# h-walk/PySlice

Hardware: AMD Instinct MI355X
Metric: slice-steps/sec (probes x frames x slices / s), potential + slice loop + exit FFT (higher is better)
Workload: dtype complex64 (f32); 1 GPU; 64-probe STEM grid, 1024x1024 grid, 200 slices, 54 MD frames per GPU (BASELINE configs[2] per-frame work), 106583 atoms, 30 mrad, 100 keV; grid=1024, slices=200, probes=64, parallelism=frames x1, world_size_checked=1, frame_slots=59, frame_batch=4

## Files before the change

pyslice_amd/csrc/mslice.hip:

```cpp
#include <hip/hip_runtime.h>

#include <algorithm>
#include <cmath>
#include <cstdarg>
#include <cstdio>
#include <cstdlib>
#include <cstring>
#include <string>
#include <vector>

#include "../../include/mslice.h"
#include "fft_generic.h"
#include "fft_pow2.h"
#include "rowtm_pass.h"
#include "potential.h"
#include "thermal.h"
#include "reduce.h"
#include "stream.h"
#include "tacaw_time.h"
#include "tacaw_launch.h"
#include "tacaw_welch.h"
#include "layer_tap.h"
#include "detect.h"
#include "spectrum_detect.h"
// ... 1196 lines not shown
    }
    switch (o.base) {
    case AX_TWO: {
        std::vector<float2> t(o.R * o.R);
        for (int m = 0; m < o.R * o.R; ++m) {
            const double a = -2.0 * M_PI * (double)m / (double)n;
            t[m] = make_float2((float)cos(a), (float)sin(a));
        }
        if ((rc = make_tw4(h, o.tw, o.R)) || (rc = upload(h, o.tw2, t)) || (rc = o.ptab.alloc(h, (size_t)n))) return rc;
        break;
    }
    case AX_WAVE2K:
        if ((rc = make_wave2k_tables(h, o.tw, o.tw2))) return rc;
        break;
    case AX_CONV:
    case AX_CONV2K:
        if ((rc = make_cz_tables(h, o.cz, n)) || (rc = o.qf.alloc(h, conv_filter_entries(o)))) return rc;
        break;
    case AX_CONV4K: {
        std::vector<float2> wq(2048);
        for (int i = 0; i < 2048; ++i) {
            const double a = -2.0 * M_PI * (double)i / 4096.0;
            wq[i] = make_float2((float)cos(a), (float)sin(a));
        }
        if ((rc = make_wave2k_tables(h, o.tw, o.tw2)) || (rc = upload(h, o.bw, wq)) || (rc = o.qf.alloc(h, conv_filter_entries(o)))) return rc;
        break;
    }
    default:
        break;
    }
    auto conv = [](const msl_handle::OpDir& d) { return d.base == AX_CONV || d.base == AX_CONV2K; };
    if (!conv(o) && conv(other) && n >= 33 && n <= 1024) return make_cz_tables(h, o.cz, n);
    return MSL_OK;
}

PotIfft plan_pot_ifft(const msl_handle* h) {
    if (!h->onepass || h->V) return PI_LINES;
    if (h->opx.base == AX_WAVE2K && h->opy.base == AX_WAVE2K && h->transT) return PI_WAVE2K;
    if (h->transT && h->opx.cz.R && h->opy.cz.R) return PI_CHIRPZ;
    if (h->opx.base == AX_TWO && h->opy.base == AX_TWO) return PI_TWO;
    return PI_LINES;
}

bool pot_half_rows(const msl_handle* h) { return h->pot_ifft != PI_LINES || (h->Rx && h->Ry); }

struct PotGroup {
    int z2s[104], species[104], nsp;
    int64_t n; int32_t ax1, ax2, axs;
    int keys_per_frame;
    int cx, cy; float vscale;
    bool half_rows, sf_stream;
    int g, slot, n_slices, nkeys;
    long long rows, rows_pad;
    float2* TR; float2* TRT;
};

int map_species(msl_handle* h, const int32_t* Z, int64_t n, PotGroup& m) {
    for (int i = 0; i < 104; ++i) m.z2s[i] = -1;
    for (int64_t a = 0; a < n; ++a) {
        if (Z[a] < 1 || Z[a] > 103) return fail(h, MSL_ERR_INVALID, "msl_build_potential: atomic number %d out of 1..103", Z[a]);
        m.z2s[Z[a]] = 0;
    }
    m.nsp = 0;
    for (int z = 1; z <= 103; ++z) if (m.z2s[z] == 0) { m.z2s[z] = m.nsp; m.species[m.nsp++] = z; }
    return MSL_OK;
}

int stage_atoms(msl_handle* h, const PotGroup& p, const double* pos, const int32_t* Z, bool send_maps) {
    msl_handle::HostStage& st = h->stage[h->stage_pos++ & 1];
    if (!st.ev) HIPCHK(h, hipEventCreateWithFlags(&st.ev, hipEventDisableTiming));
    if (st.used) HIPCHK(h, hipEventSynchronize(st.ev));
    const size_t z_bytes = (size_t)p.n * sizeof(int), pos_bytes = (size_t)p.rows * 3 * sizeof(double);
    const size_t off_sp = sizeof p.z2s, off_Z = (off_sp + sizeof p.species + 7) & ~(size_t)7;
    const size_t off_pos = (off_Z + z_bytes + 7) & ~(size_t)7, need = off_pos + pos_bytes;
    if (need > st.bytes) {
        if (st.buf) (void)hipHostFree(st.buf);
        st.buf = nullptr; st.bytes = 0;
        const size_t cap = need + need / 4;
        if (hipHostMalloc((void**)&st.buf, cap, hipHostMallocDefault) != hipSuccess)
            return fail(h, MSL_ERR_NOMEM, "hipHostMalloc(%zu bytes) failed", cap);
        st.bytes = cap;
    }
    memcpy(st.buf + off_pos, pos, pos_bytes);
    if (send_maps) {
        memcpy(st.buf, p.z2s, sizeof p.z2s);
        memcpy(st.buf + off_sp, p.species, sizeof p.species);
        memcpy(st.buf + off_Z, Z, z_bytes);
        HIPCHK(h, hipMemcpyAsync(h->d_z2s, st.buf, sizeof p.z2s, hipMemcpyHostToDevice, h->stream));
        HIPCHK(h, hipMemcpyAsync(h->d_species, st.buf + off_sp, p.nsp * sizeof(int), hipMemcpyHostToDevice, h->stream));
        HIPCHK(h, hipMemcpyAsync(h->d_Z, st.buf + off_Z, z_bytes, hipMemcpyHostToDevice, h->stream));
    }
    HIPCHK(h, hipMemcpyAsync(h->d_pos, st.buf + off_pos, pos_bytes, hipMemcpyHostToDevice, h->stream));
    HIPCHK(h, hipEventRecord(st.ev, h->stream));
    st.used = true;
    return MSL_OK;
}

struct ThermalSource { uint64_t seed; uint64_t first_config; };

int stage_thermal(msl_handle* h, const PotGroup& p, uint64_t seed, uint64_t first_config, bool send_maps) {
    if (send_maps) {
        HIPCHK(h, hipMemcpyAsync(h->d_z2s, h->th_z2s, sizeof p.z2s, hipMemcpyDeviceToDevice, h->stream));
        HIPCHK(h, hipMemcpyAsync(h->d_species, h->th_species, p.nsp * sizeof(int), hipMemcpyDeviceToDevice, h->stream));
        HIPCHK(h, hipMemcpyAsync(h->d_Z, h->th_Z, (size_t)p.n * sizeof(int), hipMemcpyDeviceToDevice, h->stream));
    }
    hipLaunchKernelGGL(thermal_positions_kernel, dim3((unsigned)((p.rows + 255) / 256)), dim3(256), 0, h->stream, h->th_pos0, h->th_sigma,
                       (long long)p.n, p.g, (unsigned long long)seed, (unsigned long long)first_config, h->d_pos);
    HIPCHK(h, hipGetLastError());
    return MSL_OK;
}

int bin_atoms(msl_handle* h, const PotGroup& p) {
    const msl_config& c = h->cfg;
    const int nsp = p.nsp;
    HIPCHK(h, hipMemsetAsync(h->d_counts, 0, ((size_t)p.nkeys + 1) * sizeof(int), h->stream));
    const double lx = c.nx * c.dx, ly = c.ny * c.dy;
    if (nsp != h->ff_n || memcmp(p.species, h->ff_species, nsp * sizeof(int)) != 0) {
        long long tot = (long long)c.nx * c.ny * nsp;
        hipLaunchKernelGGL(formfactor_kernel, dim3((unsigned)((tot + 255) / 256)), dim3(256), 0, h->stream, h->d_ff, h->d_abcd,
                           h->d_species, nsp, c.nx, c.ny, 1.0 / lx, 1.0 / ly);
        memcpy(h->ff_species, p.species, nsp * sizeof(int));
        h->ff_n = nsp;
    }
    hipLaunchKernelGGL(atom_prep_kernel, dim3((unsigned)((p.rows + 255) / 256)), dim3(256), 0, h->stream, h->d_pos, h->d_Z,
                       (long long)p.n, p.g, h->d_z2s, h->d_lo, h->d_hi, c.nz, nsp, p.ax1, p.ax2, p.axs, 1.0 / lx, 1.0 / ly, h->d_key,
                       h->d_u1, h->d_u2, h->d_counts);
    hipLaunchKernelGGL(bin_scan_kernel, dim3(1), dim3(1024), 0, h->stream, h->d_counts, h->d_start, p.nkeys, p.sf_stream ? SF_ALIGN : 1);
    hipLaunchKernelGGL(bin_fill_kernel, dim3(p.nkeys), dim3(1024), 0, h->stream, h->d_key, (long long)p.n, p.keys_per_frame, h->d_start, h->d_order);
    HIPCHK(h, hipGetLastError());
    const int* n_sorted = h->d_start + p.nkeys;
    if (p.rows_pad > 0x7fffffffLL) return fail(h, MSL_ERR_INVALID, "msl_build_potentials: %lld padded table rows in one group exceed 2^31", p.rows_pad);
    const long long tx = p.rows_pad * p.cx, ty = p.rows_pad * p.cy;
    hipLaunchKernelGGL(phase_table_kernel, dim3((unsigned)((tx + 255) / 256)), dim3(256), 0, h->stream, h->d_ex, h->d_u1,
                       h->d_order, n_sorted, c.nx, p.cx, p.cx);
    hipLaunchKernelGGL(phase_table_kernel, dim3((unsigned)((ty + 255) / 256)), dim3(256), 0, h->stream, h->d_ey, h->d_u2,
                       h->d_order, n_sorted, c.ny, p.cy, p.cy);
    return MSL_OK;
}

int launch_structure_factor(msl_handle* h, const PotGroup& p) {
    const msl_config& c = h->cfg;
    const int cx = p.cx, cy = p.cy, nsp = p.nsp, n_slices = p.n_slices, full_rows = p.half_rows ? 0 : 1;
    const bool edge_x = (c.nx % 2 == 0) && (cx % 32 == 1) && cx > 1, edge_y = (c.ny % 2 == 0) && (cy % 32 == 1) && cy > 1;
    const int tiles_x = edge_x ? cx / 32 : (cx + 31) / 32, tiles_y = edge_y ? cy / 32 : (cy + 31) / 32;
    const int n_tiles = tiles_x * tiles_y, wg_per_slice = (n_tiles + 3) / 4;
    const long long n_wg = (long long)wg_per_slice * ((n_slices + 7) / 8 * 8);
    if (n_wg > 0x7fffffffLL) return fail(h, MSL_ERR_UNSUPPORTED, "structure factor: too many workgroups");
    if (p.sf_stream) {
        const int n_pers = std::max(8, h->n_cus / 8 * 8);
        auto stream = [&](auto kernel, size_t lds, int tiles) {
            hipLaunchKernelGGL(kernel, dim3((unsigned)n_pers), dim3(256), lds, h->stream, p.TR, h->d_ex, h->d_ey, h->d_ff, h->d_start, nsp,
                               c.nx, c.ny, tiles_y, tiles, (int)p.rows_pad, full_rows, cx, cy, n_slices);
        };
        if (dbg_env("MSL_SF_F32"))
            stream(structure_factor_stream_kernel, 0, n_tiles);
        else if ((n_tiles >= 512 || (tiles_x >= 2 && dbg_env("MSL_SF_TWO_TILES"))) && !dbg_env("MSL_SF_ONE_TILE"))
            stream(structure_factor_stream_bf16x2_kernel, 4 * 128 * 64 * sizeof(float), ((tiles_x + 1) / 2) * tiles_y);
        else
            stream(structure_factor_stream_bf16_kernel, 0, n_tiles);
    } else
        hipLaunchKernelGGL(structure_factor_quad_kernel, dim3((unsigned)n_wg), dim3(256), 0, h->stream, p.TR, h->d_ex, h->d_ey, h->d_ff,
                           h->d_start, nsp, c.nx, c.ny, tiles_y, n_tiles, (int)p.rows_pad, full_rows, cx, cy, n_slices, wg_per_slice);
    if (edge_x || edge_y) {
        const int bins = (edge_x ? cy : 0) + (edge_y ? (edge_x ? cx - 1 : cx) : 0);
        for (int s0 = 0; s0 < n_slices; s0 += 65535) {
            const int ns = std::min(65535, n_slices - s0);
            hipLaunchKernelGGL(structure_factor_edge_kernel, dim3((bins + 127) / 128, ns), dim3(128), 0, h->stream,
                               p.TR + (size_t)s0 * c.nx * c.ny, h->d_ex, h->d_ey, h->d_ff, h->d_start + (size_t)s0 * nsp, nsp, c.nx, c.ny,
                               edge_x ? 1 : 0, edge_y ? 1 : 0, full_rows, cx, cy);
        }
    }
    HIPCHK(h, hipGetLastError());
    return MSL_OK;
}

int launch_ifftTW(msl_handle* h, const msl_handle::OpDir& o, IfftTBJob j) {
    constexpr int N2 = 2048;
    const size_t lds = ((size_t)N2 + 64 + (size_t)8 * (N2 + 1)) * 8;
    const long long items = (long long)(j.n_lines / 8) * j.n_images;
    const int grid = (int)std::min<long long>(items, (long long)h->n_cus);
    j.tw = o.tw; j.tw2 = o.tw2;
    return launch_lds(h, ifftTW_kernel, dim3(grid), dim3(512), lds, K_OTHER, j);
}

int launch_ifftTB(msl_handle* h, const msl_handle::OpDir& o, IfftTBJob j) {
    const CzTables& t = o.cz;
    j.tw = t.tw; j.bf = t.bf; j.bw = t.bw;
    if (t.R == 64) {
        constexpr int M2 = 2048, NH2 = 1024, RS = (32 * W2K_PITCH) / 2 + 1;
        const size_t lds2 = ((size_t)M2 + 64 + NH2 + 2 + NH2 + (size_t)8 * RS) * 8;
        const long long items2 = (long long)((j.n_lines + 7) / 8) * j.n_images;
        const int grid2 = (int)std::min<long long>(items2, (long long)h->n_cus);
        j.tw2 = t.tw2;
        return launch_lds(h, ifftTB2_kernel, dim3(grid2), dim3(512), lds2, K_OTHER, j);
    }
    const int R = t.R, M = R * R, NH = M / 2, CS = R * (R + 1) + 2;
    const size_t lds = ((size_t)M + NH + 2 + NH + (size_t)16 * CS) * 8;
    const int per_cu = std::max(1, std::min(R == 16 ? 4 : 1, (int)((size_t)h->lds_limit / lds)));
    if (R == 32 && !j.potential && !dbg_env("MSL_NO_TWO_LINE_IFFT")) {
        constexpr int CSN = 514;
        const size_t lds2 = ((size_t)M + NH + 2 + NH + (size_t)32 * CSN) * 8;
        const long long items2 = (long long)((j.n_lines + 31) / 32) * j.n_images;
        const int grid2 = (int)std::min<long long>(items2, (long long)h->n_cus);
        return launch_lds(h, ifftTB_two_kernel, dim3(grid2), dim3(512), lds2, K_OTHER, j);
    }
    const bool pair = R == 32 && j.herm && j.potential && !dbg_env("MSL_NO_PAIRED_IFFT");
    const long long items = (long long)((j.n_lines + (pair ? 31 : 15)) / (pair ? 32 : 16)) * j.n_images;
    const dim3 grid((unsigned)std::min<long long>(items, (long long)h->n_cus * per_cu));
    if (pair) return launch_lds(h, ifftTB_kernel<32, true>, grid, dim3(512), lds, K_OTHER, j);
    if (R == 32) return launch_lds(h, ifftTB_kernel<32>, grid, dim3(512), lds, K_OTHER, j);
    return launch_lds(h, ifftTB_kernel<16>, grid, dim3(256), lds, K_OTHER, j);
}

int launch_ifftT2(msl_handle* h, const msl_handle::OpDir& o, IfftT2Job j) {
    constexpr int R = 16, N2 = R * R, N = 2 * N2;
    const size_t lds = ((size_t)2 * N2 + (size_t)16 * (N + 1)) * 8;
    const int per_cu = std::max(1, std::min(2, (int)((size_t)h->lds_limit / lds)));
    const bool pair = j.herm && j.potential && j.n_lines % 32 == 0 && !dbg_env("MSL_NO_PAIRED_IFFT");
    const long long items = (long long)(j.n_lines / (pair ? 32 : 16)) * j.n_images;
    const dim3 grid((unsigned)std::min<long long>(items, (long long)h->n_cus * per_cu));
    j.tw = o.tw; j.tw2 = o.tw2;
    if (pair) return launch_lds(h, ifftT2_kernel<16, true>, grid, dim3(256), lds, K_OTHER, j);
    return launch_lds(h, ifftT2_kernel<16>, grid, dim3(256), lds, K_OTHER, j);
}

template <typename Job>
int ifft_transposed(msl_handle* h, const PotGroup& p, int line_block, int (*launch)(msl_handle*, const msl_handle::OpDir&, Job)) {
    const msl_config& c = h->cfg;
    const long long npix = (long long)c.nx * c.ny;
    Job a{};
    a.in = p.TR; a.out_t = p.TRT; a.out_rows = nullptr;
    a.in_is = a.out_t_is = npix; a.in_pitch = c.ny; a.out_t_pitch = c.nx; a.n_images = p.n_slices;
    a.n_lines = (c.nx / 2 + 1 + line_block - 1) / line_block * line_block;
    a.potential = 0; a.rows_parity = -1; a.slice_mod = c.nz;
    Job b{};
    b.in = p.TRT; b.out_t = p.TR; b.out_rows = p.TRT;
    b.in_is = b.out_t_is = b.out_rows_is = npix; b.in_pitch = c.nx; b.out_t_pitch = c.ny; b.out_rows_pitch = c.nx;
    b.n_lines = c.ny; b.n_images = p.n_slices; b.potential = 1; b.herm = 1; b.slice_mod = c.nz;
    b.rows_parity = slice_is_transposed(h, 1) ? 1 : 0;
    b.scale = p.vscale; b.sigma_over_pi = (float)(c.sigma / M_PI);
    if constexpr (std::is_same<Job, IfftTBJob>::value) { a.n_line = c.ny; b.n_line = c.nx; }
    const int rc = launch(h, h->opy, a);
    return rc ? rc : launch(h, h->opx, b);
}

int ifft_inplace(msl_handle* h, const PotGroup& p) {
    const msl_config& c = h->cfg;
    int rc;
    if (h->Ry) {
        RowJob r = row_job(h, p.TR, p.n_slices, c.ny);
        r.do_ifft = 1;
        if (p.half_rows) { const int Gr = 256 / h->Ry; r.nx = (c.nx / 2 + 1 + Gr - 1) / Gr * Gr; }
        if ((rc = launch_row_fast(h, r, K_OTHER))) return rc;
    } else {
        LineArgs r = row_args(h, p.TR, p.TR, p.n_slices, c.ny);
        r.fft1 = -1;
        if ((rc = launch_lines(h, h->plan_y, r, K_OTHER))) return rc;
    }
    if (h->Rx) {
        ColJob k = col_job(h, p.TR, p.TR, p.n_slices, c.ny, c.ny);
        k.flags = COL_INV | COL_POTENTIAL; k.scale = p.vscale; k.sigma = (float)c.sigma; k.out_real = h->V; k.slice_mod = c.nz;
        if (h->onepass && !h->V) { k.flags |= COL_TPOT; k.tparity = h->scheme_b ? 0 : ((c.nz - 1) & 1); k.out_t = p.TRT; }
        if ((rc = p.half_rows ? launch_col_herm(h, k, K_OTHER) : launch_col_fast(h, k, K_OTHER))) return rc;
        return (h->onepass && h->V) ? transpose_odd_slices(h, p.slot) : MSL_OK;
    }
    LineArgs k = col_args(h, p.TR, p.TR, p.n_slices, c.ny, c.ny);
    k.fft1 = -1; k.scale = p.vscale;
    k.store_mode = STORE_POTENTIAL; k.out_real = h->V; k.sigma = (float)c.sigma;
    if ((rc = launch_lines(h, h->plan_x, k, K_OTHER))) return rc;
    for (int f = 0; f < p.g && rc == MSL_OK; ++f) rc = transpose_odd_slices(h, p.slot + f);
    return rc;
}

int potential_ifft(msl_handle* h, const PotGroup& p) {
    h->cur = nullptr;
    switch (h->pot_ifft) {
    case PI_WAVE2K: return ifft_transposed(h, p, 8, launch_ifftTW);
    case PI_CHIRPZ: return ifft_transposed(h, p, 1, launch_ifftTB);
    case PI_TWO:    return ifft_transposed(h, p, 16, launch_ifftT2);
    default:        return ifft_inplace(h, p);
    }
}

int build_potentials(msl_handle* h, const double* pos, const int32_t* Z, int64_t n, int count, int first_slot, int32_t ax1, int32_t ax2, int32_t axs,
                     const ThermalSource* th = nullptr) {
    const msl_config& c = h->cfg;
    const size_t npix = (size_t)c.nx * c.ny;
    PotGroup p{};
    int rc = MSL_OK;
    if (th) {
        memcpy(p.z2s, h->th_map_z2s, sizeof p.z2s);
        memcpy(p.species, h->th_map_species, sizeof p.species);
        p.nsp = h->th_nsp;
    } else {
        rc = map_species(h, Z, n, p);
    }
    if (rc) return rc;
    EventPair timer;
    if (c.launch_timing && (rc = timer.begin(h))) return rc;
    if (p.nsp > h->ff_species_cap) {
        if ((rc = h->d_ff.alloc(h, npix * p.nsp))) return rc;
        h->ff_species_cap = p.nsp;
        h->ff_n = 0;
    }
    p.n = n; p.ax1 = ax1; p.ax2 = ax2; p.axs = axs;
    p.cx = c.nx / 2 + 1; p.cy = c.ny / 2 + 1; p.keys_per_frame = c.nz * std::max(p.nsp, 1);
    p.half_rows = pot_half_rows(h);
    p.sf_stream = (double)n / std::max(1, p.keys_per_frame) >= 128.0 && !dbg_env("MSL_SF_TILED");
    p.vscale = (float)(1.0 / ((double)c.nx * c.ny) / (c.dx * c.dx * c.dy * c.dy));
// ... 1803 lines not shown
```

pyslice_amd/csrc/potential.h:

```cpp
#pragma once
#include <hip/hip_runtime.h>
#include <stdint.h>
#include "kernel_util.h"

namespace msl {

__device__ __forceinline__ int signed_freq(int m, int n) { return (m < (n + 1) / 2) ? m : m - n; }

__global__ void formfactor_kernel(float* __restrict__ ff, const double* __restrict__ abcd,
                                  const int* __restrict__ species, int n_species, int nx, int ny,
                                  double inv_lx, double inv_ly) {
    long long i = (long long)blockIdx.x * blockDim.x + threadIdx.x;
    long long npix = (long long)nx * ny;
    if (i >= npix * n_species) return;
    int sp = (int)(i / npix);
    long long p = i - (long long)sp * npix;
    int mx = (int)(p / ny), my = (int)(p - (long long)mx * ny);
    double kx = signed_freq(mx, nx) * inv_lx, ky = signed_freq(my, ny) * inv_ly;
    double q2 = kx * kx + ky * ky;
    const double* t = abcd + (size_t)(species[sp] - 1) * 12;
    double s1 = 0.0, s2 = 0.0;
#pragma unroll
    for (int j = 0; j < 3; ++j) {
        s1 += t[j * 4 + 0] / (q2 + t[j * 4 + 1]);
// ... 349 lines not shown
                x[u] = make_float2(a.x, a.y); y[u] = make_float2(b.x, b.y);
            }
        };
        auto mma = [&](f32x16& acc, const sf_u32x4& a, const sf_u32x4& b) { asm volatile("v_mfma_f32_32x32x16_bf16 %0, %1, %2, %0" : "+a"(acc) : "v"(a), "v"(b)); };
        auto mma6 = [&](f32x16& acc, const sf_u32x4 (&p)[3], const sf_u32x4 (&q)[3]) {
            mma(acc, p[0], q[0]); mma(acc, p[0], q[1]); mma(acc, p[1], q[0]);
            mma(acc, p[0], q[2]); mma(acc, p[2], q[0]); mma(acc, p[1], q[1]);
        };
        auto conv = [&](sf_u32x4 (&o)[3], const float2 (&v)[8], bool imag) {
#pragma unroll
            for (int u = 0; u < 4; ++u) {
                unsigned p0, p1, p2;
                sf_split3(imag ? v[2 * u].y : v[2 * u].x, imag ? v[2 * u + 1].y : v[2 * u + 1].x, p0, p1, p2);
                o[0][u] = p0; o[1][u] = p1; o[2][u] = p2;
            }
        };
        sf_u32x4 cx[3], sx[3], cy[3], sy[3];
        auto trip = [&](int h, float2 (&x)[8], float2 (&y)[8], const float2 (&xn)[8], const float2 (&yn)[8]) {
            if (S0 + 16 * h == seg1) flush();
            mma6(A, cx, cy); conv(sy, y, true); conv(sx, x, true); __builtin_amdgcn_sched_barrier(0);
            load16(h + 2, x, y); __builtin_amdgcn_sched_barrier(0);
            mma6(C, cx, sy); conv(cx, xn, false); __builtin_amdgcn_sched_barrier(0);
            mma6(D, sx, cy); conv(cy, yn, false); __builtin_amdgcn_sched_barrier(0);
            mma6(B, sx, sy); __builtin_amdgcn_sched_barrier(0);
        };
        float2 x0[8], y0[8], x1[8], y1[8];
        if (H > 0) { load16(0, x0, y0); load16(1, x1, y1); conv(cx, x0, false); conv(cy, y0, false); }
        for (int h = 0; h < H; h += 2) {
            trip(h, x0, y0, x1, y1);
            if (h + 1 < H) trip(h + 1, x1, y1, x0, y0);
        }
        if (H > 0) flush();
        float2* out = recip + (size_t)s * nx * ny;
        const int my = ky0 + i;
        if (my > hy) continue;
#pragma unroll
        for (int r = 0; r < 16; ++r) {
            const int mx = kx0 + (r & 3) + 8 * (r >> 2) + 4 * kk;
            if (mx > hx) continue;
            store_quad_bin(out, nx, ny, mx, my, tA[r], tB[r], tC[r], tD[r], write_mx);
        }
    }
}

__global__ void __launch_bounds__(256, 1) structure_factor_stream_bf16x2_kernel(float2* __restrict__ recip, const float2* __restrict__ ex,
                                                                             const float2* __restrict__ ey, const float* __restrict__ ff,
                                                                             const int* __restrict__ start, int n_species, int nx, int ny,
                                                                             int tiles_y, int n_pairs, int n_rows, int write_mx, int px_pitch,
                                                                             int py_pitch, int n_slices) {
    extern __shared__ float sf_tot[];
    const int xcd = blockIdx.x & 7, jw = blockIdx.x >> 3, wg_x = gridDim.x >> 3;
    const int lane = threadIdx.x & 63, wave = threadIdx.x >> 6;
    const int hx = nx / 2, hy = ny / 2;
    const int i = lane & 31, kk = lane >> 5;
    const int G = (n_pairs + 3) / 4, Mx = (n_slices + 7) / 8;
    for (int q = jw; q < Mx * G; q += wg_x) {
        const int m = q / G, g = q - m * G;
        const int s = xcd + 8 * m, pair = 4 * g + wave;
        if (s >= n_slices || pair >= n_pairs) continue;
        const int kx0 = (pair / tiles_y) * 64, ky0 = (pair % tiles_y) * 32;
        const int lx0 = min(kx0 + i, hx), lx1 = min(kx0 + 32 + i, hx), ly = min(ky0 + i, hy);
        const int* st = start + s * n_species;
        const int S0 = __builtin_amdgcn_readfirstlane(st[0]), S1 = __builtin_amdgcn_readfirstlane(st[n_species]);
        const int H = (S1 - S0) >> 4;
        const unsigned rows_left = (unsigned)(n_rows - S0);
        const msl_i4v rx = make_raw_rsrc(ex + (size_t)S0 * px_pitch, (unsigned)((unsigned long long)rows_left * px_pitch * 8ull < 0xfffffff0ull ? (unsigned long long)rows_left * px_pitch * 8ull : 0xfffffff0ull));
        const msl_i4v ry = make_raw_rsrc(ey + (size_t)S0 * py_pitch, (unsigned)((unsigned long long)rows_left * py_pitch * 8ull < 0xfffffff0ull ? (unsigned long long)rows_left * py_pitch * 8ull : 0xfffffff0ull));
        const int vox0 = (8 * kk * px_pitch + lx0) * 8, vox1 = (8 * kk * px_pitch + lx1) * 8, voy = (8 * kk * py_pitch + ly) * 8;
        f32x16 A0, B0, C0, D0, A1, B1, C1, D1;
        const sf_u32x4 z4 = {0u, 0u, 0u, 0u};
        auto zero_acc = [&](f32x16& acc) { asm volatile("s_nop 15\n\ts_nop 15\n\tv_mfma_f32_32x32x16_bf16 %0, %1, %1, 0\n\ts_nop 15\n\ts_nop 15" : "=a"(acc) : "v"(z4)); };
        zero_acc(A0); zero_acc(B0); zero_acc(C0); zero_acc(D0); zero_acc(A1); zero_acc(B1); zero_acc(C1); zero_acc(D1);
        float* tot = sf_tot + (wave * 128) * 64 + lane;
#pragma unroll
        for (int r = 0; r < 128; ++r) tot[r * 64] = 0.f;
        int sp = -1, seg1 = S0;
        auto next_of = [&](int& k, int& e) { const int from = e; do { ++k; if (k >= n_species) return; e = st[k + 1]; } while (e <= from); };
        float w0[16], w1[16];
        auto load_w = [&](int spc) {
            const float* f = ff + (size_t)spc * nx * ny;
#pragma unroll
            for (int r = 0; r < 16; ++r) {
                const int row = (r & 3) + 8 * (r >> 2) + 4 * kk;
                w0[r] = f[(size_t)min(kx0 + row, hx) * ny + ly];
                w1[r] = f[(size_t)min(kx0 + 32 + row, hx) * ny + ly];
            }
        };
#pragma unroll
        for (int r = 0; r < 16; ++r) { w0[r] = 0.f; w1[r] = 0.f; }
        next_of(sp, seg1);
        if (sp < n_species) load_w(sp);
        auto flush = [&]() {
            asm volatile("s_nop 15\n\ts_nop 15\n\ts_nop 15\n\ts_nop 15\n\ts_nop 15\n\ts_nop 15" ::: "memory");
#pragma unroll
            for (int r = 0; r < 16; ++r) {
                float* t = tot + r * 64;
                t[0 * 1024] = fmaf(w0[r], A0[r], t[0 * 1024]); t[1 * 1024] = fmaf(w0[r], B0[r], t[1 * 1024]);
                t[2 * 1024] = fmaf(w0[r], C0[r], t[2 * 1024]); t[3 * 1024] = fmaf(w0[r], D0[r], t[3 * 1024]);
                t[4 * 1024] = fmaf(w1[r], A1[r], t[4 * 1024]); t[5 * 1024] = fmaf(w1[r], B1[r], t[5 * 1024]);
                t[6 * 1024] = fmaf(w1[r], C1[r], t[6 * 1024]); t[7 * 1024] = fmaf(w1[r], D1[r], t[7 * 1024]);
            }
            zero_acc(A0); zero_acc(B0); zero_acc(C0); zero_acc(D0); zero_acc(A1); zero_acc(B1); zero_acc(C1); zero_acc(D1);
            next_of(sp, seg1);
            if (sp < n_species) load_w(sp);
        };
        auto load16 = [&](int h, float2 (&xa)[8], float2 (&xb)[8], float2 (&y)[8]) {
            const int r0 = __builtin_amdgcn_readfirstlane(16 * h);
#pragma unroll
            for (int u = 0; u < 8; ++u) {
                const msl_f2v a = msl_raw_buffer_load_f2(rx, vox0, (r0 + u) * px_pitch * 8, 0);
                const msl_f2v c = msl_raw_buffer_load_f2(rx, vox1, (r0 + u) * px_pitch * 8, 0);
                const msl_f2v b = msl_raw_buffer_load_f2(ry, voy, (r0 + u) * py_pitch * 8, 0);
                xa[u] = make_float2(a.x, a.y); xb[u] = make_float2(c.x, c.y); y[u] = make_float2(b.x, b.y);
            }
        };
        auto mma = [&](f32x16& acc, const sf_u32x4& a, const sf_u32x4& b) { asm volatile("v_mfma_f32_32x32x16_bf16 %0, %1, %2, %0" : "+a"(acc) : "v"(a), "v"(b)); };
        auto mma6 = [&](f32x16& acc, const sf_u32x4 (&p)[3], const sf_u32x4 (&qq)[3]) {
            mma(acc, p[0], qq[0]); mma(acc, p[0], qq[1]); mma(acc, p[1], qq[0]);
            mma(acc, p[0], qq[2]); mma(acc, p[2], qq[0]); mma(acc, p[1], qq[1]);
        };
        auto conv = [&](sf_u32x4 (&o)[3], const float2 (&v)[8], bool imag) {
#pragma unroll
            for (int u = 0; u < 4; ++u) {
                unsigned p0, p1, p2;
                sf_split3(imag ? v[2 * u].y : v[2 * u].x, imag ? v[2 * u + 1].y : v[2 * u + 1].x, p0, p1, p2);
                o[0][u] = p0; o[1][u] = p1; o[2][u] = p2;
            }
        };
        sf_u32x4 cx0[3], sx0[3], cx1[3], sx1[3], cy[3], sy[3];
        auto trip = [&](int h, float2 (&xa)[8], float2 (&xb)[8], float2 (&y)[8], const float2 (&xan)[8], const float2 (&xbn)[8], const float2 (&yn)[8]) {
            if (S0 + 16 * h == seg1) flush();
            mma6(A0, cx0, cy); mma6(A1, cx1, cy); conv(sy, y, true); conv(sx0, xa, true); conv(sx1, xb, true); __builtin_amdgcn_sched_barrier(0);
            load16(h + 2, xa, xb, y); __builtin_amdgcn_sched_barrier(0);
            mma6(C0, cx0, sy); mma6(C1, cx1, sy); conv(cx0, xan, false); conv(cx1, xbn, false); __builtin_amdgcn_sched_barrier(0);
            mma6(D0, sx0, cy); mma6(D1, sx1, cy); conv(cy, yn, false); __builtin_amdgcn_sched_barrier(0);
            mma6(B0, sx0, sy); mma6(B1, sx1, sy); __builtin_amdgcn_sched_barrier(0);
        };
        float2 xa0[8], xb0[8], y0[8], xa1[8], xb1[8], y1[8];
        if (H > 0) { load16(0, xa0, xb0, y0); load16(1, xa1, xb1, y1); conv(cx0, xa0, false); conv(cx1, xb0, false); conv(cy, y0, false); }
        for (int h = 0; h < H; h += 2) {
            trip(h, xa0, xb0, y0, xa1, xb1, y1);
            if (h + 1 < H) trip(h + 1, xa1, xb1, y1, xa0, xb0, y0);
        }
        if (H > 0) flush();
        float2* out = recip + (size_t)s * nx * ny;
        const int my = ky0 + i;
        if (my > hy) continue;
#pragma unroll
        for (int r = 0; r < 16; ++r) {
            const int mx = kx0 + (r & 3) + 8 * (r >> 2) + 4 * kk;
            const float* t = tot + r * 64;
            if (mx <= hx) store_quad_bin(out, nx, ny, mx, my, t[0 * 1024], t[1 * 1024], t[2 * 1024], t[3 * 1024], write_mx);
            if (mx + 32 <= hx) store_quad_bin(out, nx, ny, mx + 32, my, t[4 * 1024], t[5 * 1024], t[6 * 1024], t[7 * 1024], write_mx);
        }
    }
}


__global__ void __launch_bounds__(128) structure_factor_edge_kernel(float2* __restrict__ recip, const float2* __restrict__ ex,
                                                                    const float2* __restrict__ ey, const float* __restrict__ ff,
                                                                    const int* __restrict__ start, int n_species, int nx, int ny,
                                                                    int edge_x, int edge_y, int write_mx, int px_pitch, int py_pitch) {
    const int s = blockIdx.y;
    const int hx = nx / 2, hy = ny / 2;
    const int n_row = edge_x ? hy + 1 : 0;
    const int n_col = edge_y ? (edge_x ? hx : hx + 1) : 0;
    const int i = blockIdx.x * blockDim.x + threadIdx.x;
    if (i >= n_row + n_col) return;
    const int mx = i < n_row ? hx : i - n_row, my = i < n_row ? i : hy;
    float tA = 0.f, tB = 0.f, tC = 0.f, tD = 0.f;
    for (int sp = 0; sp < n_species; ++sp) {
        const int a0 = start[s * n_species + sp], a1 = start[s * n_species + sp + 1];
        float A = 0.f, B = 0.f, C = 0.f, D = 0.f;
        int a = a0;
        for (; a + 8 <= a1; a += 8) {
            float2 x[8], y[8];
#pragma unroll
            for (int u = 0; u < 8; ++u) { x[u] = ex[(size_t)(a + u) * px_pitch + mx]; y[u] = ey[(size_t)(a + u) * py_pitch + my]; }
#pragma unroll
            for (int u = 0; u < 8; ++u) {
                A = fmaf(x[u].x, y[u].x, A); B = fmaf(x[u].y, y[u].y, B); C = fmaf(x[u].x, y[u].y, C); D = fmaf(x[u].y, y[u].x, D);
            }
        }
        for (; a < a1; ++a) {
            const float2 x = ex[(size_t)a * px_pitch + mx], y = ey[(size_t)a * py_pitch + my];
            A = fmaf(x.x, y.x, A); B = fmaf(x.y, y.y, B); C = fmaf(x.x, y.y, C); D = fmaf(x.y, y.x, D);
        }
        const float w = ff[(size_t)sp * nx * ny + (size_t)mx * ny + my];
        tA = fmaf(w, A, tA); tB = fmaf(w, B, tB); tC = fmaf(w, C, tC); tD = fmaf(w, D, tD);
    }
    store_quad_bin(recip + (size_t)s * nx * ny, nx, ny, mx, my, tA, tB, tC, tD, write_mx);
}

__global__ void probe_kspace_kernel(float2* __restrict__ psik, const double* __restrict__ xy, int P, int nx, int ny,
                                    int pitch, double inv_lx, double inv_ly, double kfreq_x, double kfreq_y, double radius,
                                    int plane_wave) {
    long long i = (long long)blockIdx.x * blockDim.x + threadIdx.x;
    long long npix = (long long)nx * ny;
    if (i >= npix * P) return;
    int p = (int)(i / npix);
    long long q = i - (long long)p * npix;
    int mx = (int)(q / ny), my = (int)(q - (long long)mx * ny);
    const long long o = ((long long)p * nx + mx) * pitch + my;
    if (plane_wave) {
        psik[o] = (mx == 0 && my == 0) ? make_float2((float)npix, 0.f) : make_float2(0.f, 0.f);
        return;
    }
    int fx = signed_freq(mx, nx), fy = signed_freq(my, ny);
    double kx = fx * kfreq_x, ky = fy * kfreq_y;
    bool inside = sqrt(kx * kx + ky * ky) < radius;
    if (!inside) { psik[o] = make_float2(0.f, 0.f); return; }
    double t = fx * ((double)(nx / 2) / nx + xy[2 * p] * inv_lx) + fy * ((double)(ny / 2) / ny + xy[2 * p + 1] * inv_ly);
    t -= rint(t);
    float sn, cs;
    sincospif((float)(2.0 * t), &sn, &cs);
    psik[o] = make_float2(cs, sn);
}

struct ProbeAberrations {
    double a[14], b[14];
};

__global__ void probe_kspace_aberr_kernel(float2* __restrict__ psik, const double* __restrict__ xy, int P, int nx, int ny,
                                          int pitch, double inv_lx, double inv_ly, double kfreq_x, double kfreq_y, double radius,
                                          double wavelength, ProbeAberrations ab) {
    long long i = (long long)blockIdx.x * blockDim.x + threadIdx.x;
    long long npix = (long long)nx * ny;
    if (i >= npix * P) return;
    int p = (int)(i / npix);
    long long q = i - (long long)p * npix;
    int mx = (int)(q / ny), my = (int)(q - (long long)mx * ny);
    const long long o = ((long long)p * nx + mx) * pitch + my;
    int fx = signed_freq(mx, nx), fy = signed_freq(my, ny);
    double kx = fx * kfreq_x, ky = fy * kfreq_y;
    bool inside = sqrt(kx * kx + ky * ky) < radius;
    if (!inside) { psik[o] = make_float2(0.f, 0.f); return; }
    double t = fx * ((double)(nx / 2) / nx + xy[2 * p] * inv_lx) + fy * ((double)(ny / 2) / ny + xy[2 * p + 1] * inv_ly);
    const double ax = wavelength * kx, ay = wavelength * ky;
    const double r2 = fma(ax, ax, ay * ay);
    const double c2 = fma(ax, ax, -ay * ay), s2 = 2.0 * ax * ay;
    const double c3 = fma(c2, ax, -s2 * ay), s3 = fma(c2, ay, s2 * ax);
    const double c4 = fma(c3, ax, -s3 * ay), s4 = fma(c3, ay, s3 * ax);
    const double c5 = fma(c4, ax, -s4 * ay), s5 = fma(c4, ay, s4 * ax);
    const double c6 = fma(c5, ax, -s5 * ay), s6 = fma(c5, ay, s5 * ax);
    double chi = r2 * fma(r2, fma(r2, ab.a[10], ab.a[4]), ab.a[0]);
    chi = fma(ax, r2 * fma(r2, ab.a[7], ab.a[2]), chi);
    chi = fma(ay, r2 * fma(r2, ab.b[7], ab.b[2]), chi);
    chi = fma(c2, fma(r2, fma(r2, ab.a[11], ab.a[5]), ab.a[1]), chi);
    chi = fma(s2, fma(r2, fma(r2, ab.b[11], ab.b[5]), ab.b[1]), chi);
    chi = fma(c3, fma(r2, ab.a[8], ab.a[3]), chi);
    chi = fma(s3, fma(r2, ab.b[8], ab.b[3]), chi);
    chi = fma(c4, fma(r2, ab.a[12], ab.a[6]), chi);
    chi = fma(s4, fma(r2, ab.b[12], ab.b[6]), chi);
    chi = fma(c5, ab.a[9], chi);
    chi = fma(s5, ab.b[9], chi);
    chi = fma(c6, ab.a[13], chi);
    chi = fma(s6, ab.b[13], chi);
    t -= chi;
    t -= rint(t);
    float sn, cs;
    sincospif((float)(2.0 * t), &sn, &cs);
    psik[o] = make_float2(cs, sn);
}

__global__ void probe_ramp_kernel(float2* __restrict__ out, const float2* __restrict__ basek,
                                  const double* __restrict__ xy, int P, int nx, int ny, int pitch, double inv_lx, double inv_ly) {
    long long i = (long long)blockIdx.x * blockDim.x + threadIdx.x;
    long long npix = (long long)nx * ny;
    if (i >= npix * P) return;
    int p = (int)(i / npix);
    long long q = i - (long long)p * npix;
    int mx = (int)(q / ny), my = (int)(q - (long long)mx * ny);
    const long long o = ((long long)p * nx + mx) * pitch + my;
    double t = signed_freq(mx, nx) * (xy[2 * p] * inv_lx) + signed_freq(my, ny) * (xy[2 * p + 1] * inv_ly);
    t -= rint(t);
    float sn, cs;
    sincospif((float)(2.0 * t), &sn, &cs);
    float2 b = basek[q];
    out[o] = make_float2(b.x * cs - b.y * sn, b.x * sn + b.y * cs);
}

__global__ void transmission_kernel(float2* __restrict__ t, const float* __restrict__ V, long long n, float sigma) {
    long long i = (long long)blockIdx.x * blockDim.x + threadIdx.x;
    if (i >= n) return;
    float sn, cs;
    sincosf(sigma * V[i], &sn, &cs);
    t[i] = make_float2(cs, sn);
}

}
```

Measured before the change: 240,900 slice-steps/s.

## Add quad-tile bf16 MFMA structure-factor stream kernel with species rescaling

Adds a persistent structure-factor kernel in which each wave computes a 2x2 block of 32x32 tiles (64x64 bins). Loaded x and y phase rows and their bf16 splits are reused across four accumulators, which raises MFMA work per global load. Species segments are handled by rescaling the accumulators by a form-factor ratio at each boundary, so per-species form factors are no longer applied per atom row. The new kernel becomes the default whenever there are at least two tiles in each direction. It holds 64 accumulator vectors per lane, which raises register pressure, and the ratio rescaling can lose precision or divide by zero if a form-factor value is near zero.

```diff
diff --git a/pyslice_amd/csrc/mslice.hip b/pyslice_amd/csrc/mslice.hip
--- a/pyslice_amd/csrc/mslice.hip
+++ b/pyslice_amd/csrc/mslice.hip
@@ -1372,9 +1372,13 @@
             hipLaunchKernelGGL(kernel, dim3((unsigned)n_pers), dim3(256), lds, h->stream, p.TR, h->d_ex, h->d_ey, h->d_ff, h->d_start, nsp,
                                c.nx, c.ny, tiles_y, tiles, (int)p.rows_pad, full_rows, cx, cy, n_slices);
         };
+        const bool one_tile = dbg_env("MSL_SF_ONE_TILE"), two_tiles = dbg_env("MSL_SF_TWO_TILES");
         if (dbg_env("MSL_SF_F32"))
             stream(structure_factor_stream_kernel, 0, n_tiles);
-        else if ((n_tiles >= 512 || (tiles_x >= 2 && dbg_env("MSL_SF_TWO_TILES"))) && !dbg_env("MSL_SF_ONE_TILE"))
+        else if (!one_tile && !two_tiles && ((tiles_x >= 2 && tiles_y >= 2) || dbg_env("MSL_SF_QUAD_TILES")))
+            hipLaunchKernelGGL(structure_factor_stream_bf16q_kernel, dim3((unsigned)n_pers), dim3(256), 0, h->stream, p.TR, h->d_ex, h->d_ey, h->d_ff,
+                               h->d_start, nsp, c.nx, c.ny, tiles_x, tiles_y, (int)p.rows_pad, full_rows, cx, cy, n_slices);
+        else if ((n_tiles >= 512 || (tiles_x >= 2 && two_tiles)) && !one_tile)
             stream(structure_factor_stream_bf16x2_kernel, 4 * 128 * 64 * sizeof(float), ((tiles_x + 1) / 2) * tiles_y);
         else
             stream(structure_factor_stream_bf16_kernel, 0, n_tiles);
diff --git a/pyslice_amd/csrc/potential.h b/pyslice_amd/csrc/potential.h
--- a/pyslice_amd/csrc/potential.h
+++ b/pyslice_amd/csrc/potential.h
@@ -525,6 +525,143 @@
             const float* t = tot + r * 64;
             if (mx <= hx) store_quad_bin(out, nx, ny, mx, my, t[0 * 1024], t[1 * 1024], t[2 * 1024], t[3 * 1024], write_mx);
             if (mx + 32 <= hx) store_quad_bin(out, nx, ny, mx + 32, my, t[4 * 1024], t[5 * 1024], t[6 * 1024], t[7 * 1024], write_mx);
+        }
+    }
+}
+
+typedef __bf16 sf_bf16x8 __attribute__((ext_vector_type(8)));
+__device__ float msl_raw_buffer_load_f1(msl_i4v rsrc, int voffset, int soffset, int aux) __asm("llvm.amdgcn.raw.buffer.load.f32");
+__global__ void __launch_bounds__(256, 1) structure_factor_stream_bf16q_kernel(float2* __restrict__ recip, const float2* __restrict__ ex,
+                                                                            const float2* __restrict__ ey, const float* __restrict__ ff,
+                                                                            const int* __restrict__ start, int n_species, int nx, int ny,
+                                                                            int tiles_x, int tiles_y, int n_rows, int write_mx, int px_pitch,
+                                                                            int py_pitch, int n_slices) {
+    const int xcd = blockIdx.x & 7, jw = blockIdx.x >> 3, wg_x = gridDim.x >> 3;
+    const int lane = threadIdx.x & 63, wave = threadIdx.x >> 6;
+    const int hx = nx / 2, hy = ny / 2;
+    const int x_end = min(hx + 1, 32 * tiles_x), y_end = min(hy + 1, 32 * tiles_y);
+    const int i = lane & 31, kk = lane >> 5;
+    const int blocks_x = (tiles_x + 1) / 2, blocks_y = (tiles_y + 1) / 2;
+    const int gx_n = (blocks_x + 1) / 2, gy_n = (blocks_y + 1) / 2;
+    const int G = gx_n * gy_n, Mx = (n_slices + 7) / 8;
+    for (int q = jw; q < Mx * G; q += wg_x) {
+        const int m = q / G, g = q - m * G;
+        const int s = xcd + 8 * m;
+        const int gy = g / gx_n, gx = g - gy * gx_n;
+        const int bx = 2 * gx + (wave >> 1), by = 2 * gy + (wave & 1);
+        if (s >= n_slices || bx >= blocks_x || by >= blocks_y) continue;
+        const int kx0 = bx * 64, ky0 = by * 64;
+        const int lx0 = min(kx0 + i, hx), lx1 = min(kx0 + 32 + i, hx), ly0 = min(ky0 + i, hy), ly1 = min(ky0 + 32 + i, hy);
+        const int* st = start + s * n_species;
+        const int S0 = __builtin_amdgcn_readfirstlane(st[0]), S1 = __builtin_amdgcn_readfirstlane(st[n_species]);
+        const int H = (S1 - S0) >> 4;
+        const unsigned rows_left = (unsigned)(n_rows - S0);
+        const msl_i4v rx = make_raw_rsrc(ex + (size_t)S0 * px_pitch, (unsigned)((unsigned long long)rows_left * px_pitch * 8ull < 0xfffffff0ull ? (unsigned long long)rows_left * px_pitch * 8ull : 0xfffffff0ull));
+        const msl_i4v ry = make_raw_rsrc(ey + (size_t)S0 * py_pitch, (unsigned)((unsigned long long)rows_left * py_pitch * 8ull < 0xfffffff0ull ? (unsigned long long)rows_left * py_pitch * 8ull : 0xfffffff0ull));
+        const int vox0 = (8 * kk * px_pitch + lx0) * 8, vox1 = (8 * kk * px_pitch + lx1) * 8;
+        const int voy0 = (8 * kk * py_pitch + ly0) * 8, voy1 = (8 * kk * py_pitch + ly1) * 8;
+        f32x16 acc[2][2][4];
+#pragma unroll
+        for (int t = 0; t < 16; ++t)
+#pragma unroll
+            for (int r = 0; r < 16; ++r) acc[t >> 3][(t >> 2) & 1][t & 3][r] = 0.f;
+        const int vow0 = ((kx0 + 4 * kk) * ny + ly0) * 4, vow1 = ((kx0 + 4 * kk) * ny + ly1) * 4;
+        auto load_w = [&](int spc, int tx, int ty, float (&o)[16]) {
+            const msl_i4v rw = make_raw_rsrc(ff + (size_t)spc * nx * ny, (unsigned)nx * (unsigned)ny * 4u);
+#pragma unroll
+            for (int r = 0; r < 16; ++r) o[r] = msl_raw_buffer_load_f1(rw, ty ? vow1 : vow0, (32 * tx + (r & 3) + 8 * (r >> 2)) * ny * 4, 0);
+        };
+        int sp = -1, seg1 = S0;
+        auto next_of = [&](int& k, int& e) { const int from = e; do { ++k; if (k >= n_species) return; e = st[k + 1]; } while (e <= from); };
+        next_of(sp, seg1);
+        auto boundary = [&]() {
+            const int spc = sp;
+            next_of(sp, seg1);
+            if (sp >= n_species) { sp = spc; return; }
+#pragma unroll
+            for (int t = 0; t < 4; ++t) {
+                const int tx = t >> 1, ty = t & 1;
+                float wc[16], wn[16];
+                load_w(spc, tx, ty, wc);
+                load_w(sp, tx, ty, wn);
+#pragma unroll
+                for (int r = 0; r < 16; ++r) {
+                    const float f = wc[r] / wn[r];
+#pragma unroll
+                    for (int p = 0; p < 4; ++p) acc[tx][ty][p][r] *= f;
+                }
+            }
+        };
+        float2 x0[8], x1[8], y0[8], y1[8];
+        auto load16x = [&](int h) {
+            const int r0 = __builtin_amdgcn_readfirstlane(16 * h);
+#pragma unroll
+            for (int u = 0; u < 8; ++u) {
+                const msl_f2v a = msl_raw_buffer_load_f2(rx, vox0, (r0 + u) * px_pitch * 8, 0);
+                const msl_f2v c = msl_raw_buffer_load_f2(rx, vox1, (r0 + u) * px_pitch * 8, 0);
+                x0[u] = make_float2(a.x, a.y); x1[u] = make_float2(c.x, c.y);
+            }
+        };
+        auto load16y = [&](int h) {
+            const int r0 = __builtin_amdgcn_readfirstlane(16 * h);
+#pragma unroll
+            for (int u = 0; u < 8; ++u) {
+                const msl_f2v b = msl_raw_buffer_load_f2(ry, voy0, (r0 + u) * py_pitch * 8, 0);
+                const msl_f2v d = msl_raw_buffer_load_f2(ry, voy1, (r0 + u) * py_pitch * 8, 0);
+                y0[u] = make_float2(b.x, b.y); y1[u] = make_float2(d.x, d.y);
+            }
+        };
+        auto conv = [&](sf_u32x4 (&o)[3], const float2 (&v)[8], bool imag) {
+#pragma unroll
+            for (int u = 0; u < 4; ++u) {
+                unsigned p0, p1, p2;
+                sf_split3(imag ? v[2 * u].y : v[2 * u].x, imag ? v[2 * u + 1].y : v[2 * u + 1].x, p0, p1, p2);
+                o[0][u] = p0; o[1][u] = p1; o[2][u] = p2;
+            }
+        };
+        auto mma = [&](f32x16& c, const sf_u32x4& a, const sf_u32x4& b) {
+            c = __builtin_amdgcn_mfma_f32_32x32x16_bf16(__builtin_bit_cast(sf_bf16x8, a), __builtin_bit_cast(sf_bf16x8, b), c, 0, 0, 0);
+        };
+        auto mma6 = [&](f32x16& c, const sf_u32x4 (&p)[3], const sf_u32x4 (&qq)[3]) {
+            mma(c, p[0], qq[0]); mma(c, p[0], qq[1]); mma(c, p[1], qq[0]);
+            mma(c, p[0], qq[2]); mma(c, p[2], qq[0]); mma(c, p[1], qq[1]);
+        };
+        if (H > 0) { load16x(0); load16y(0); }
+        for (int h = 0; h < H;) {
+          const int h_end = min(H, (__builtin_amdgcn_readfirstlane(seg1) - S0) >> 4);
+          for (; h < h_end; ++h) {
+            sf_u32x4 cx0[3], sx0[3], cx1[3], sx1[3], cy0[3], sy0[3], cy1[3], sy1[3];
+            conv(cx0, x0, false); conv(cy0, y0, false); __builtin_amdgcn_sched_barrier(0);
+            mma6(acc[0][0][0], cx0, cy0); conv(cx1, x1, false); conv(cy1, y1, false); __builtin_amdgcn_sched_barrier(0);
+            mma6(acc[1][0][0], cx1, cy0); mma6(acc[0][1][0], cx0, cy1); conv(sy0, y0, true); conv(sy1, y1, true); __builtin_amdgcn_sched_barrier(0);
+            load16y(h + 1); __builtin_amdgcn_sched_barrier(0);
+            mma6(acc[1][1][0], cx1, cy1); mma6(acc[0][0][2], cx0, sy0); conv(sx0, x0, true); conv(sx1, x1, true); __builtin_amdgcn_sched_barrier(0);
+            load16x(h + 1); __builtin_amdgcn_sched_barrier(0);
+            mma6(acc[1][0][2], cx1, sy0); mma6(acc[0][1][2], cx0, sy1); mma6(acc[1][1][2], cx1, sy1);
+            mma6(acc[0][0][3], sx0, cy0); mma6(acc[0][1][3], sx0, cy1); mma6(acc[1][0][3], sx1, cy0); mma6(acc[1][1][3], sx1, cy1);
+            mma6(acc[0][0][1], sx0, sy0); mma6(acc[0][1][1], sx0, sy1);
+            mma6(acc[1][0][1], sx1, sy0); mma6(acc[1][1][1], sx1, sy1); __builtin_amdgcn_sched_barrier(0);
+          }
+          if (h < H) boundary();
+        }
+        float2* out = recip + (size_t)s * nx * ny;
+#pragma unroll
+        for (int t = 0; t < 4; ++t) {
+            const int tx = t >> 1, ty = t & 1;
+            const int my = ky0 + 32 * ty + i;
+            if (my >= y_end) continue;
+            float wl[16];
+#pragma unroll
+            for (int r = 0; r < 16; ++r) wl[r] = 0.f;
+            if (H > 0) load_w(sp, tx, ty, wl);
+#pragma unroll
+            for (int r = 0; r < 16; ++r) {
+                const int mx = kx0 + 32 * tx + (r & 3) + 8 * (r >> 2) + 4 * kk;
+                if (mx >= x_end) continue;
+                const float f = wl[r];
+                store_quad_bin(out, nx, ny, mx, my, f * acc[tx][ty][0][r], f * acc[tx][ty][1][r], f * acc[tx][ty][2][r], f * acc[tx][ty][3][r],
+                               write_mx);
+            }
         }
     }
 }
```

Measured after the change: 241,700 slice-steps/s, median of 6. Within noise of the previous version (+0.4%).
